# zouyilin2000/pockit

Measured on AMD Instinct MI355X. Metric: NLP-callback cycles/sec (f + grad f + g + J + H), higher is better.
Workload: dtype f64; 1 GPU; planar_quadrotor LGR 2000 intervals x 6 points (12000 nodes; n=96008, m=96000, nnz_J=755925, nnz_H=359972); inputs=guess*(1+1e-3 U) seed 0; lambda N(0,1) seed 1; sigma 1

## Files before the change

__graft_entry__.py:

```python
import os
import sys

ROOT = os.path.dirname(os.path.abspath(__file__))
if ROOT not in sys.path:
    sys.path.insert(0, ROOT)


def _bench_models():
    from pockit_amd import benchmarks as models
    import pockit_amd.radau as radau

    yield models.brachistochrone(radau, 3, 4)
    yield models.brachistochrone(radau, 200, 8)
    yield models.planar_quadrotor(radau, 2000, 6)
    yield models.two_stage_rocket(radau, 1000, 4)
    yield models.humanoid_wbc(radau, 50, 8)
    import pockit_amd.lobatto as lobatto

    yield models.planar_quadrotor(lobatto, 20, 6)
    yield models.three_stage_rocket(radau, 1000, 4)
    yield models.humanoid_team(radau, 5000, 8)


def _batch_models():
    from pockit_amd import benchmarks as models
    import pockit_amd.lobatto as lobatto
    import pockit_amd.radau as radau

    yield models.brachistochrone(radau, 3, 4)
    yield models.brachistochrone(radau, 60, 5)
    yield models.two_stage_rocket(radau, 6, 4)
    yield models.planar_quadrotor(lobatto, 20, 6)


def build() -> None:
    from pockit_amd import hipbuild, runtime
    from pockit_amd.codegen import ModelSource

    hipbuild.build_runtime(force=True)
    lib = runtime.load_library()
    for name in runtime.EXPORTS:
        getattr(lib, name)
    from pockit_amd.evaluator import compile_batched, compile_plan

    for system, _, _ in _batch_models():
        src, _ = compile_plan(system.plan)
        compile_batched(system.plan, src)
    for k, (system, _, _) in enumerate(_bench_models()):
        compile_plan(system.plan)
        if k in (2, 3, 4):
            hipbuild.compile_model(ModelSource(system.plan, sharded=True).source, fastmath=system._fastmath)
    import oracle.radau
    import subprocess

    subprocess.run([sys.executable, os.path.join(ROOT, "tools", "prune_cache.py")], check=False)


def smoke() -> None:
    import numpy as np

    from pockit_amd import benchmarks as models
    import oracle.radau
    import pockit_amd.radau as radau

    system, _, guess = models.brachistochrone(radau, 6, 5)
    ref, _, ref_guess = models.brachistochrone(oracle.radau, 6, 5)
    x, lam, sigma = models.bench_inputs(system, guess)

    def close(a, b):
        a, b = np.asarray(a), np.asarray(b)
        assert a.shape == b.shape
        assert np.max(np.abs(a - b)) <= 1e-11 * max(1.0, np.max(np.abs(b))), np.max(np.abs(a - b))

    close(system.objective(x), ref.objective(x))
    close(system.gradient(x), ref.gradient(x))
    close(system.constraints(x), ref.constraints(x))
    close(system.jacobian(x), ref.jacobian(x))
    close(system.hessian(x, lam, sigma), ref.hessian(x, lam, sigma))
    jr, jc = system.jacobianstructure()
    rr, rc = ref.jacobianstructure()
    assert np.array_equal(jr, rr) and np.array_equal(jc, rc)
    print("smoke OK: f, grad f, g, J, H of brachistochrone LGR 6x5 match the oracle on", "cuda:0")


if __name__ == "__main__":
    build()
    if len(sys.argv) > 1 and sys.argv[1] == "smoke":
        smoke()
```

pockit_amd/csrc/pk_kernels.hip.h:

```cpp
#pragma once
#include <hip/hip_runtime.h>
#include "pk_abi.h"

struct PkSys {
  const double* s;
  const double* I;
  double sigma;
  const double* lams;
};

namespace pk {

template <int G>
struct Grp {};

#define PK_CONST_AS __attribute__((address_space(4)))
typedef const int64_t PK_CONST_AS* pk_cbase_t;
__device__ __forceinline__ pk_cbase_t const_bases(const int64_t* p) { return (pk_cbase_t)(uintptr_t)p; }
__device__ __forceinline__ PkTile load_tile(const PkTile* p) {
  const int32_t PK_CONST_AS* src = (const int32_t PK_CONST_AS*)(uintptr_t)p;
  PkTile t;
  int32_t* dst = reinterpret_cast<int32_t*>(&t);
#pragma unroll
  for (int k = 0; k < (int)(sizeof(PkTile) / sizeof(int32_t)); ++k) dst[k] = src[k];
  return t;
}

template <int N>
struct SegBases {
  int lo, hi;
  pk_cbase_t mem;
  __device__ __forceinline__ void load(const int64_t* __restrict__ lb, int off, int lane) {
    mem = const_bases(lb + off);
    if (N <= PK_WAVE) {
      const long long v = lane < N ? (long long)lb[off + lane] : 0ll;
      lo = (int)v;
      hi = (int)(v >> 32);
    }
  }
  __device__ __forceinline__ void settle() {
    if (N <= PK_WAVE) asm volatile("" : "+v"(lo), "+v"(hi));
  }
  __device__ __forceinline__ int64_t operator[](int e) const {
    if (N > PK_WAVE) return mem[e];
    const unsigned l = (unsigned)__builtin_amdgcn_readlane(lo, e), h = (unsigned)__builtin_amdgcn_readlane(hi, e);
    return (int64_t)(((unsigned long long)h << 32) | l);
  }
};

template <int N>
__device__ __forceinline__ void settle(double (&v)[N]) {
#pragma unroll
  for (int i = 0; i < N; ++i) asm volatile("" : "+v"(v[i]));
}

template <int N>
__device__ __forceinline__ void fresh_args(double (&a)[N], double& tau, double& dt, double& w) {
  settle(a);
  asm volatile("" : "+v"(tau), "+v"(w));
  (void)dt;
}

__device__ __forceinline__ void loads_done() { __builtin_amdgcn_s_waitcnt(0x0F70); }

__device__ __forceinline__ void wave_lds_sync() {
  __builtin_amdgcn_fence(__ATOMIC_RELEASE, "wavefront");
  __builtin_amdgcn_wave_barrier();
  __builtin_amdgcn_fence(__ATOMIC_ACQUIRE, "wavefront");
}

#define PK_NPHASE_DIM (PK_NPHASE > 0 ? PK_NPHASE : 1)
#define PK_XCDS 8
__device__ __forceinline__ int xcd_ids_below(int n, int y) { return (n + PK_XCDS - 1 - y) / PK_XCDS; }
__device__ __forceinline__ int xcd_tile_block(int wg, int first, int total) {
  const int x = wg % PK_XCDS;
  int start = 0;
#pragma unroll
  for (int y = 0; y < PK_XCDS; ++y)
    if (y < x) start += xcd_ids_below(total, y) - xcd_ids_below(first, y);
  return start + xcd_ids_below(wg, x) - xcd_ids_below(first, x);
}

#ifdef PK_TRACE
#define PK_DIAG(bits) ((A.flags & (bits)) != 0)
#else
#define PK_DIAG(bits) false
#endif
#ifdef PK_TRACE
#define PK_TRACE_REC(role) const int pk_trec = tl.pad >= 0 ? tl.pad * 3 + (role) : -1
#define PK_MARK_AT(rec, k)                                                                                   \
  do {                                                                                                      \
    if (A.trace != nullptr && (threadIdx.x & 63) == 0 && (rec) >= 0)                                        \
      A.trace[(size_t)(rec) * 16 + (k)] = __builtin_amdgcn_s_memrealtime();                                 \
  } while (0)
#define PK_MARK(k) PK_MARK_AT(pk_trec, k)
#define PK_TRACE_PARAM , int pk_trec
#define PK_TRACE_ARG , pk_trec
#else
#define PK_TRACE_PARAM
#define PK_TRACE_ARG
#define PK_TRACE_REC(role) do { } while (0)
#define PK_MARK_AT(rec, k) do { } while (0)
#define PK_MARK(k) do { } while (0)
#endif

#ifndef PK_STREAM_FLAGS
#define PK_STREAM_FLAGS "sc1"
#endif

__device__ __forceinline__ void put(double* __restrict__ p, double v) {
  __hip_atomic_store(p, v, __ATOMIC_RELAXED, __HIP_MEMORY_SCOPE_AGENT);
}

template <int CTRL, int ROW_MASK>
__device__ __forceinline__ double dpp_take(double v) {
  const int lo = __builtin_amdgcn_update_dpp(0, __double2loint(v), CTRL, ROW_MASK, 0xf, false);
  const int hi = __builtin_amdgcn_update_dpp(0, __double2hiint(v), CTRL, ROW_MASK, 0xf, false);
  return __hiloint2double(hi, lo);
}

__device__ __forceinline__ double wave_sum(double v) {
  v += dpp_take<0xb1, 0xf>(v);
  v += dpp_take<0x4e, 0xf>(v);
  v += dpp_take<0x114, 0xf>(v);
  v += dpp_take<0x118, 0xf>(v);
  v += dpp_take<0x142, 0xa>(v);
  v += dpp_take<0x143, 0xc>(v);
  const int lo = __builtin_amdgcn_readlane(__double2loint(v), 63);
  const int hi = __builtin_amdgcn_readlane(__double2hiint(v), 63);
  return __hiloint2double(hi, lo);
}

template <int N>
__device__ __forceinline__ void wave_sums_to(double* v, double* __restrict__ dst, int lane) {
  if constexpr (N > 0) {
#pragma unroll
    for (int r = 0; r < N; ++r) v[r] = wave_sum(v[r]);
    if (lane == 0) {
#pragma unroll
      for (int r = 0; r < N; ++r) dst[r] = v[r];
    }
  }
}

#ifndef PK_BIG_MFMA
#define PK_BIG_MFMA 0
#endif
typedef double pk_d4 __attribute__((ext_vector_type(4)));
template <class Store>
__device__ __forceinline__ void mfma_rows(const double* __restrict__ Amat, int lda, int nrows, int kdim, double scale,
                                          const double* __restrict__ Bcol, int ldb, int ncols, int rb, int cb, int lane,
                                          Store&& store) {
  pk_d4 acc = {0.0, 0.0, 0.0, 0.0};
  const int arow = rb * 16 + (lane & 15), bcol = cb * 16 + (lane & 15), kq = lane >> 4;
  const bool a_ok = arow < nrows, b_ok = bcol < ncols;
  const double* __restrict__ ap = Amat + (size_t)(a_ok ? arow : 0) * lda;
  const double* __restrict__ bp = Bcol + (size_t)(b_ok ? bcol : 0) * ldb;
  for (int k0 = 0; k0 < kdim; k0 += 64) {
    double a4[4][4];
#pragma unroll
    for (int g = 0; g < 4; ++g)
#pragma unroll
      for (int u = 0; u < 4; ++u) {
        const int k = k0 + 16 * g + 4 * kq + u;
        a4[g][u] = (a_ok && k < kdim) ? ap[k] : 0.0;
      }
#pragma unroll
    for (int g = 0; g < 4; ++g) {
      if (k0 + 16 * g >= kdim) break;
      double b4[4];
#pragma unroll
      for (int u = 0; u < 4; ++u) {
        const int k = k0 + 16 * g + 4 * kq + u;
        b4[u] = (b_ok && k < kdim) ? bp[k] : 0.0;
      }
#pragma unroll
      for (int u = 0; u < 4; ++u) acc = __builtin_amdgcn_mfma_f64_16x16x4f64(a4[g][u] * scale, b4[u], acc, 0, 0, 0);
    }
  }
  if (b_ok) {
#pragma unroll
    for (int reg = 0; reg < 4; ++reg) {
      const int r = rb * 16 + kq + 4 * reg;
      if (r < nrows) store(r, bcol, acc[reg]);
    }
  }
}

#define PK_POLL_SLEEP 4
#define PK_POLL_LIMIT (1 << 24)
__device__ __forceinline__ void handoff_put(unsigned long long* slot, double v) {
  unsigned long long b = (unsigned long long)__double_as_longlong(v);
  if (b == PK_EMPTY) b = 0x7FF8000000000000ull;
  __hip_atomic_store(slot, b, __ATOMIC_RELAXED, __HIP_MEMORY_SCOPE_AGENT);
}
// ... 161 lines not shown
                                           double* acc) {
  double a[K];
#pragma unroll
  for (int c = 0; c < K; ++c) a[c] = full[c] * width * 0.5;
#pragma unroll
  for (int c = 0; c < K; ++c) {
#pragma unroll
    for (int i = 0; i < P::NX; ++i) acc[i] += a[c] * f[i * PK_WAVE + c];
  }
}

template <class P>
__device__ __forceinline__ void defect_loop(const double* __restrict__ full, const double* __restrict__ f, double width,
                                            double* acc, int K) {
#pragma unroll 4
  for (int c = 0; c < K; ++c) {
    const double a = full[c] * width * 0.5;
#pragma unroll
    for (int i = 0; i < P::NX; ++i) acc[i] += a * f[i * PK_WAVE + c];
  }
}
template <class P, int K>
__device__ __forceinline__ void defect_dot_k(const double* __restrict__ full, const double* __restrict__ f, double width,
                                             double* acc) {
  if constexpr (K * P::NX <= PK_DOT_UNROLL_MAX) defect_dot<P, K>(full, f, width, acc);
  else defect_loop<P>(full, f, width, acc, K);
}

template <class P, bool STAGED>
__device__ __forceinline__ void write_defects(const PkArgs& A, const PkPhase& ph, const PkTile& tl,
                                              const TileGeom& g, const TileTabs& T, const double* s, double dt,
                                              const double* __restrict__ fsv, const double* xr, double* xe,
                                              int lane) {
  const int nrows = tl.nj * g.R;
  if (lane >= nrows) return;
  const int jj = magic_div((uint32_t)lane, tl.magicR), r = lane - jj * g.R;
  const int endslot = tl.q0 + (jj + 1) * g.stride;
  const int back_slot = P::SCHEME ? ph.L_m - 1 : ph.L_m;
  const double* __restrict__ f = fsv + jj * g.stride;
  double acc[P::NX];
#pragma unroll
  for (int i = 0; i < P::NX; ++i) acc[i] = 0.0;
  if (STAGED) {
    const double width = T.wd[jj];
    const double* __restrict__ full = T.full + r * g.K;
    switch (g.K) {
      case 1: defect_dot_k<P, 1>(full, f, width, acc); break;
      case 2: defect_dot_k<P, 2>(full, f, width, acc); break;
      case 3: defect_dot_k<P, 3>(full, f, width, acc); break;
      case 4: defect_dot_k<P, 4>(full, f, width, acc); break;
      case 5: defect_dot_k<P, 5>(full, f, width, acc); break;
      case 6: defect_dot_k<P, 6>(full, f, width, acc); break;
      case 7: defect_dot_k<P, 7>(full, f, width, acc); break;
      case 8: defect_dot_k<P, 8>(full, f, width, acc); break;
      default:
        defect_loop<P>(full, f, width, acc, g.K);
        break;
    }
  } else {
    const double* __restrict__ full = A.db + tl.full_off + r * g.K;
    const double width = A.db[ph.width_off + tl.j0 + jj];
#pragma unroll 4
    for (int c = 0; c < g.K; ++c) {
      const double a = full[c] * width * 0.5;
#pragma unroll
      for (int i = 0; i < P::NX; ++i) acc[i] += a * f[i * PK_WAVE + c];
    }
  }
#pragma unroll
  for (int i = 0; i < P::NX; ++i) {
    if (endslot == back_slot) xe[i] = P::back_value(i, xe[i], s);
    put(&A.o_g[ph.g_off + i * ph.L_d + tl.r0 + lane], (xr[i] - xe[i]) - acc[i] * dt);
  }
}

#define PK_WIDE_NX 16
template <class P, bool STAGED, int I0, int CN, int ROW0 = I0>
__device__ __forceinline__ void defect_chunk(const PkArgs& A, const PkPhase& ph, const PkTile& tl, const TileGeom& g,
                                             const TileTabs& T, const double* s, double dt, const double* __restrict__ fsv,
                                             const double* a, int lane) {
  const int nrows = tl.nj * g.R;
  const int jj = min(magic_div((uint32_t)lane, tl.magicR), max(tl.nj - 1, 0)), r = lane - jj * g.R;
  const int src = (jj + 1) * g.stride;
  double xe[CN];
#pragma unroll
  for (int e = 0; e < CN; ++e) xe[e] = __shfl(a[I0 + e], src & (PK_WAVE - 1), PK_WAVE);
  if (lane >= nrows) return;
  if (src >= PK_WAVE) {
    const double* __restrict__ xp = A.x + ph.x_off;
#pragma unroll
    for (int e = 0; e < CN; ++e) xe[e] = xp[(I0 + e) * ph.state_len + tl.q0 + src];
  }
  const int endslot = tl.q0 + src;
  const int back_slot = P::SCHEME ? ph.L_m - 1 : ph.L_m;
  const double* __restrict__ f = fsv + jj * g.stride;
  const double* __restrict__ full = STAGED ? T.full + r * g.K : A.db + tl.full_off + r * g.K;
  const double width = STAGED ? T.wd[jj] : A.db[ph.width_off + tl.j0 + jj];
  double acc[CN];
#pragma unroll
  for (int e = 0; e < CN; ++e) acc[e] = 0.0;
#pragma unroll 4
  for (int c = 0; c < g.K; ++c) {
    const double wc = full[c] * width * 0.5;
#pragma unroll
    for (int e = 0; e < CN; ++e) acc[e] += wc * f[(ROW0 + e) * PK_WAVE + c];
  }
#pragma unroll
  for (int e = 0; e < CN; ++e) {
    if (endslot == back_slot) xe[e] = P::back_value(I0 + e, xe[e], s);
    put(&A.o_g[ph.g_off + (I0 + e) * ph.L_d + tl.r0 + lane], (a[I0 + e] - xe[e]) - acc[e] * dt);
  }
}
#define PK_TRANS_CHUNK 16
template <class P, bool STAGED, int I0>
__device__ __forceinline__ void write_translation_wide(const PkArgs& A, const PkTile& tl, const TileTabs& T,
                                                       const SegBases<P::NX>& tbase, int lane) {
  if constexpr (I0 < P::NX) {
    constexpr int CN = P::NX - I0 < PK_TRANS_CHUNK ? P::NX - I0 : PK_TRANS_CHUNK;
    const int tot = tl.nj * tl.nnzT;
    const double* __restrict__ tvg = A.db + tl.tv_off;
    double* __restrict__ run[CN];
    if constexpr (P::NX > PK_WAVE) {
      pk_cbase_t tb = tbase.mem + I0;
      asm volatile("" : "+s"(tb));
#pragma unroll
      for (int i = 0; i < CN; ++i) run[i] = A.o_jac + (tb[i] + tl.offT);
    } else {
#pragma unroll
      for (int i = 0; i < CN; ++i) run[i] = A.o_jac + (tbase[I0 + i] + tl.offT);
    }
    for (uint32_t p = lane; p < (uint32_t)tot; p += PK_WAVE) {
      const int t = (int)p - magic_div(p, tl.magicT) * tl.nnzT;
      const double v = STAGED ? T.tv[t] : tvg[t];
#pragma unroll
      for (int i = 0; i < CN; ++i) put(&run[i][p], v);
    }
    write_translation_wide<P, STAGED, I0 + PK_TRANS_CHUNK>(A, tl, T, tbase, lane);
  }
}
template <class P, bool STAGED>
__device__ __forceinline__ void write_translation(const PkArgs& A, const PkPhase& ph, const PkTile& tl,
                                                  const TileTabs& T, const SegBases<P::NX>& tbase, int lane) {
  if constexpr (P::NX > PK_WIDE_NX) return write_translation_wide<P, STAGED, 0>(A, tl, T, tbase, lane);
  const int tot = tl.nj * tl.nnzT;
  const double* __restrict__ tvg = A.db + tl.tv_off;
  double* __restrict__ run[P::NX];
#pragma unroll
  for (int i = 0; i < P::NX; ++i) run[i] = A.o_jac + (tbase[i] + tl.offT);
  for (uint32_t p = lane; p < (uint32_t)tot; p += PK_WAVE) {
    const int t = (int)p - magic_div(p, tl.magicT) * tl.nnzT;
    const double v = STAGED ? T.tv[t] : tvg[t];
#pragma unroll
    for (int i = 0; i < P::NX; ++i) put(&run[i][p], v);
  }
}

template <class P, int NI, bool HESS, bool STAGED, int E0, int S0, class Bases>
__device__ __forceinline__ void stream_loop(const PkArgs& A, const PkPhase& ph, const PkTile& tl, const TileGeom& g,
                                            const TileTabs& T, const double* __restrict__ sv,
                                            const double* __restrict__ lam_s, const Bases& bases,
                                            double* __restrict__ out, int lane) {
  double* __restrict__ run[NI > 0 ? NI : 1];
#pragma unroll
  for (int e = 0; e < NI; ++e) run[e] = out + (bases[E0 + e] + tl.offI);
  const int nnz = tl.nnzI;
  const int tot = tl.nj * nnz;
  if (STAGED) {
    typedef double pk_d2 __attribute__((ext_vector_type(2)));
    for (uint32_t p0 = 2 * lane; p0 < (uint32_t)tot; p0 += 2 * PK_WAVE) {
      double v[2][NI > 0 ? NI : 1];
      const bool pair = p0 + 1 < (uint32_t)tot;
#pragma unroll
      for (int u = 0; u < 2; ++u) {
        const uint32_t pc = (u == 0 || pair) ? p0 + u : p0;
        const int jj = magic_div(pc, tl.magicI);
        const int t = (int)pc - jj * nnz;
        const int rc = T.rc[t];
        const double val = -(T.iv[t] * T.wd[jj] * 0.5);
        const double* __restrict__ col = sv + jj * g.stride + (rc >> 16);
        const double* __restrict__ lam = lam_s + jj * g.R + (rc & 0xFFFF);
#pragma unroll
        for (int e = 0; e < NI; ++e)
          v[u][e] = HESS ? val * lam[(P::H_state(E0 + e) - S0) * PK_WAVE] * col[e * PK_WAVE] : val * col[e * PK_WAVE];
      }
#pragma unroll
      for (int e = 0; e < NI; ++e) {
        if (pair) {
          const pk_d2 w = {v[0][e], v[1][e]};
          asm volatile("global_store_dwordx4 %0, %1, off " PK_STREAM_FLAGS "\n\ts_nop 1" : : "v"(&run[e][p0]), "v"(w));
        } else {
          put(&run[e][p0], v[0][e]);
        }
      }
    }
    return;
  }
  const int32_t* __restrict__ rcg = A.ib + tl.irc_off;
  const double* __restrict__ ivg = A.db + tl.iv_off;
  const double* __restrict__ wdg = A.db + ph.width_off + tl.j0;
  for (uint32_t p = lane; p < (uint32_t)tot; p += PK_WAVE) {
    const int jj = magic_div(p, tl.magicI);
    const int t = (int)p - jj * nnz;
    const int r = rcg[2 * t], c = rcg[2 * t + 1];
    const double val = -(ivg[t] * wdg[jj] * 0.5);
    const double* __restrict__ col = sv + jj * g.stride + c;
    if (HESS) {
      const double* __restrict__ lam = lam_s + jj * g.R + r;
#pragma unroll
      for (int e = 0; e < NI; ++e) put(&run[e][p], val * lam[(P::H_state(E0 + e) - S0) * PK_WAVE] * col[e * PK_WAVE]);
    } else {
#pragma unroll
      for (int e = 0; e < NI; ++e) put(&run[e][p], val * col[e * PK_WAVE]);
    }
  }
}

template <class P, int NI, bool HESS, bool STAGED, int E0 = 0, int S0 = 0, class Bases>
__device__ __forceinline__ void stream_expanded(const PkArgs& A, const PkPhase& ph, const PkTile& tl,
                                                const TileGeom& g, const TileTabs& T, const double* __restrict__ sv,
                                                const double* __restrict__ lam_s, const Bases& segb,
                                                double* __restrict__ out, int lane) {
  if (NI == 0 || tl.nj * tl.nnzI == 0) return;
  stream_loop<P, NI, HESS, STAGED, E0, S0>(A, ph, tl, g, T, sv, lam_s, segb, out, lane);
}

#define PK_PHASE_B(T, CALL)       \
  do {                            \
    if ((T).staged) {             \
      constexpr bool STAGED = true;  \
      CALL;                       \
    } else {                      \
      constexpr bool STAGED = false; \
      CALL;                       \
    }                             \
  } while (0)

template <class P>
__device__ __forceinline__ void node_gradient_eval(const PkPhase& ph, int q, const double* a, double tau, double dt,
                                                   double w, const PkSys& sy, double* ov, double* orr, bool have_mid) {
  if (q == 0)
    P::front_grad(a, tau, dt, w, sy, nullptr, ov, orr);
  else if (P::SCHEME == 1 && q == ph.L_m - 1)
    P::back_grad(a, tau, dt, w, sy, nullptr, ov, orr);
  else if (!have_mid)
    P::mid_grad(a, tau, dt, w, sy, nullptr, ov, orr);
}

template <class P>
__device__ __forceinline__ void node_gradient_store(const PkArgs& A, const PkPhase& ph, int q, const double* ov) {
  double* __restrict__ gp = A.o_grad + ph.x_off;
#pragma unroll
  for (int i = 0; i < P::NX; ++i) put(&gp[i * ph.state_len + q], ov[i]);
#pragma unroll
  for (int i = 0; i < P::NU; ++i) put(&gp[P::NX * ph.state_len + i * ph.L_m + q], ov[P::NX + i]);
}

template <class P>
__device__ __forceinline__ void node_gradient(const PkArgs& A, const PkPhase& ph, int q, const double* a,
                                              double tau, double dt, double w, const PkSys& sy, double* ov,
                                              double* orr, bool have_mid) {
  node_gradient_eval<P>(ph, q, a, tau, dt, w, sy, ov, orr, have_mid);
  node_gradient_store<P>(A, ph, q, ov);
}

template <class P>
__device__ __forceinline__ void tile_int(const PkArgs& A, const PkTile& tl, double* __restrict__,
                                         double* __restrict__ wint, double* __restrict__, int lane) {
  if (P::INT_N == 0) return;
  const PkPhase& ph = A.ph[P::INDEX];
  const TileGeom g = tile_geom<P>(tl);
  double s[PK_NS], dt, mt;
  phase_scalars<P>(A, ph, s, dt, mt);
  double o[P::INT_N > 0 ? P::INT_N : 1];
#pragma unroll
  for (int r = 0; r < P::INT_N; ++r) o[r] = 0.0;
  if (lane < g.nown) {
    double a[P::NARG], tau, w;
    load_node<P>(A, ph, s, dt, mt, tl.q0 + lane, a, tau, w);
    P::mid_int(a, o);
#pragma unroll
    for (int r = 0; r < P::INT_N; ++r) o[r] *= w;
  }
  wave_sums_to<P::INT_N>(o, wint, lane);
}

template <class P, int C>
__device__ __forceinline__ void dyn_pass(const PkArgs& A, const PkPhase& ph, const PkTile& tl, const TileGeom& g,
                                         const TileTabs& T, const double* s, double dt, double mt,
                                         double* __restrict__ sv, int lane) {
  constexpr int I0 = P::D_c0(C), CN = P::D_cn(C);
  double a[P::NARG], tau, w;
  load_node<P>(A, ph, s, dt, mt, tl.q0 + lane, a, tau, w);
  if (lane < g.nq) {
    double o[CN];
    P::mid_dyn_g(Grp<C>{}, a, o);
#pragma unroll
    for (int e = 0; e < CN; ++e) sv[e * PK_WAVE + lane] = o[e];
  }
  wave_lds_sync();
  PK_PHASE_B(T, (defect_chunk<P, STAGED, I0, CN, 0>(A, ph, tl, g, T, s, dt, sv, a, lane)));
}
template <class P, int C = 0>
__device__ __forceinline__ void dyn_passes(const PkArgs& A, const PkPhase& ph, const PkTile& tl, const TileGeom& g,
                                           const TileTabs& T, const double* s, double dt, double mt,
                                           double* __restrict__ sv, int lane) {
  if constexpr (C < P::D_NG) {
// ... 475 lines not shown
  PK_MARK(4);
  wave_lds_sync();
  PK_MARK(5);
  if (tl.nj == 0) return;
  PK_PHASE_B(T, (stream_expanded<P, P::H_NI, true, STAGED, 0, S0>(A, ph, tl, g, T, sv, lam_s, segb, A.o_hess, lane)));
  PK_MARK(8);
#ifdef PK_TRACE
  __builtin_amdgcn_s_waitcnt(0);
  PK_MARK(9);
#endif
}

template <class P, int G>
__device__ __forceinline__ void hess_rows(const PkArgs& A, const PkPhase& ph, const PkTile& tl, double* __restrict__ lam_s,
                                          int lane) {
  constexpr int S0 = P::H_gs0(G), SN = P::H_gsn(G);
  if constexpr (P::H_gni(G) > 0 && SN > 0) {
    const int row = min(tl.r0 + lane, ph.L_d - 1);
    double lrow[SN];
#pragma unroll
    for (int i = 0; i < SN; ++i) lrow[i] = A.lam[ph.g_off + (S0 + i) * ph.L_d + row];
#pragma unroll
    for (int i = 0; i < SN; ++i) lam_s[i * PK_WAVE + lane] = lrow[i];
  }
}
template <class P, int G, bool STAGED>
__device__ __forceinline__ void hess_group_b(const PkArgs& A, const PkPhase& ph, const PkTile& tl, const TileGeom& g,
                                             const TileTabs& T, const double* __restrict__ sv,
                                             const double* __restrict__ lam_s, const SegBases<P::H_NI + P::H_NN>& segb,
                                             int lane) {
  stream_expanded<P, P::H_gni(G), true, STAGED, P::H_gi0(G), P::H_gs0(G)>(A, ph, tl, g, T, sv, lam_s, segb, A.o_hess, lane);
}
template <class P, int G, bool ONE = false>
__device__ __forceinline__ void hess_groups(const PkArgs& A, const PkPhase& ph, const PkTile& tl, const TileGeom& g,
                                            const TileTabs& T, double (&a)[P::NARG], double& tau, double& dt, double& w,
                                            const PkSys& sy, double (&lp)[P::NC > 0 ? P::NC : 1], double* __restrict__ sv,
                                            double* __restrict__ lam_s, const SegBases<P::H_NI + P::H_NN>& segb,
                                            int lane, int q, bool live, const double* s = nullptr, double mt = 0.0) {
  if constexpr (G < P::H_NG) {
    constexpr int NI = P::H_gni(G), N0 = P::H_gn0(G), NN = P::H_gnn(G);
    if constexpr (P::WIDE && !ONE) {
      hess_rows<P, G>(A, ph, tl, lam_s, lane);
      load_node<P>(A, ph, s, dt, mt, q, a, tau, w);
#pragma unroll
      for (int j = 0; j < P::NC; ++j) lp[j] = A.lam[ph.path_off + j * ph.L_m + min(q, ph.L_m - 1)];
    } else if constexpr (G > 0 && !ONE) {
      fresh_args(a, tau, dt, w);
      settle(lp);
    }
    if (live) {
      double o[NI + NN + 1];
      P::mid_hess_g(Grp<G>{}, a, tau, dt, w, sy, lp, o);
#pragma unroll
      for (int e = 0; e < NI; ++e) sv[e * PK_WAVE + lane] = o[e];
      if (NN > 0 && lane < g.nown && q >= ph.mid_lo && q < ph.mid_hi) {
#pragma unroll
        for (int e = 0; e < NN; ++e) put(&A.o_hess[segb[P::H_NI + N0 + e] + (q - ph.mid_lo)], o[NI + e]);
      }
    }
    if constexpr (NI > 0) {
      wave_lds_sync();
      if (tl.nj != 0) PK_PHASE_B(T, (hess_group_b<P, G, STAGED>(A, ph, tl, g, T, sv, lam_s, segb, lane)));
      if constexpr (!ONE) wave_lds_sync();
    }
    if constexpr (!ONE) hess_groups<P, G + 1>(A, ph, tl, g, T, a, tau, dt, w, sy, lp, sv, lam_s, segb, lane, q, live, s, mt);
  }
}

template <class P>
__device__ __forceinline__ void tile_hess_grouped(const PkArgs& A, const PkTile& tl, double* __restrict__ sv, int lane) {
  const PkPhase& ph = A.ph[P::INDEX];
  const TileGeom g = tile_geom<P>(tl);
  double s[PK_NS], dt, mt;
  phase_scalars<P>(A, ph, s, dt, mt);
  const PkSys sy{s, A.Ibuf, A.sigma, A.lam};
  SegBases<P::H_NI + P::H_NN> segb;
  segb.load(A.lb, ph.hseg_off, lane);
  double* __restrict__ lam_s = sv + P::H_GMAX * PK_WAVE;
  const bool fit = tabs_fit(A, tl, g);
  const TabRegs tr = tabs_issue(A, ph, tl, g, fit, lane);
  const int q = tl.q0 + lane;
  double a[P::NARG], tau, w, lp[P::NC > 0 ? P::NC : 1];
  if constexpr (P::WIDE) {
    const TileTabs T = tabs_commit(A, tl, g, tr, fit, lane);
    segb.settle();
    loads_done();
    wave_lds_sync();
    hess_groups<P, 0>(A, ph, tl, g, T, a, tau, dt, w, sy, lp, sv, lam_s, segb, lane, q, lane < g.nq, s, mt);
  } else {
    double lrow[P::NX];
    const int row = min(tl.r0 + lane, ph.L_d - 1);
#pragma unroll
    for (int i = 0; i < P::NX; ++i) lrow[i] = A.lam[ph.g_off + i * ph.L_d + row];
    load_node<P>(A, ph, s, dt, mt, q, a, tau, w);
#pragma unroll
    for (int j = 0; j < P::NC; ++j) lp[j] = A.lam[ph.path_off + j * ph.L_m + min(q, ph.L_m - 1)];
    const TileTabs T = tabs_commit(A, tl, g, tr, fit, lane);
#pragma unroll
    for (int i = 0; i < P::NX; ++i) lam_s[i * PK_WAVE + lane] = lrow[i];
    segb.settle();
    loads_done();
    hess_groups<P, 0>(A, ph, tl, g, T, a, tau, dt, w, sy, lp, sv, lam_s, segb, lane, q, lane < g.nq);
  }
}

template <class P>
__device__ __forceinline__ void tile_hess(const PkArgs& A, const PkTile& tl, double* __restrict__ sv,
                                          double* __restrict__, double* __restrict__, int lane) {
  if constexpr (P::H_NG == 1) tile_hess_single<P>(A, tl, sv, lane);
  else tile_hess_grouped<P>(A, tl, sv, lane);
}

template <class P, int G>
__device__ __forceinline__ void tile_hess_one(const PkArgs& A, const PkTile& tl, double* __restrict__ sv, int lane) {
  const PkPhase& ph = A.ph[P::INDEX];
  const TileGeom g = tile_geom<P>(tl);
  double s[PK_NS], dt, mt;
  phase_scalars<P>(A, ph, s, dt, mt);
  const PkSys sy{s, A.Ibuf, A.sigma, A.lam};
  SegBases<P::H_NI + P::H_NN> segb;
  segb.load(A.lb, ph.hseg_off, lane);
  double* __restrict__ lam_s = sv + P::H_GMAX * PK_WAVE;
  const bool fit = tabs_fit(A, tl, g);
  const TabRegs tr = tabs_issue(A, ph, tl, g, fit, lane);
  const int q = tl.q0 + lane;
  constexpr int S0 = P::H_gs0(G), SN = P::H_gsn(G);
  double a[P::NARG], tau, w, lp[P::NC > 0 ? P::NC : 1], lrow[SN > 0 ? SN : 1];
  const int row = min(tl.r0 + lane, ph.L_d - 1);
  constexpr bool needs_rows = P::H_gni(G) > 0;
  if (needs_rows) {
#pragma unroll
    for (int i = 0; i < SN; ++i) lrow[i] = A.lam[ph.g_off + (S0 + i) * ph.L_d + row];
  }
  load_node<P>(A, ph, s, dt, mt, q, a, tau, w);
#pragma unroll
  for (int j = 0; j < P::NC; ++j) lp[j] = A.lam[ph.path_off + j * ph.L_m + min(q, ph.L_m - 1)];
  const TileTabs T = tabs_commit(A, tl, g, tr, fit, lane);
  if (needs_rows) {
#pragma unroll
    for (int i = 0; i < SN; ++i) lam_s[i * PK_WAVE + lane] = lrow[i];
  }
  segb.settle();
  loads_done();
  hess_groups<P, G, true>(A, ph, tl, g, T, a, tau, dt, w, sy, lp, sv, lam_s, segb, lane, q, lane < g.nq);
}
template <class P, int G = 0>
__device__ __forceinline__ void tile_hess_pick(int grp, const PkArgs& A, const PkTile& tl, double* __restrict__ sv, int lane) {
  if constexpr (G < P::H_NG) {
    if (grp == G) tile_hess_one<P, G>(A, tl, sv, lane);
    else tile_hess_pick<P, G + 1>(grp, A, tl, sv, lane);
  }
}

template <class P, int ROLE, bool STAGED, bool CJ>
__device__ __forceinline__ void xall_phase_b(const PkArgs& A, const PkPhase& ph, const PkTile& tl, const TileGeom& g,
                                             const TileTabs& T, const double* s, double dt,
                                             const double* __restrict__ sv, const double* __restrict__ jsv,
                                             const double* xr, double* xe,
                                             const SegBases<P::J_NI + P::J_NN>& segb, const SegBases<P::NX>& tbase,
                                             int lane PK_TRACE_PARAM) {
  if (ROLE != 2 && !PK_DIAG(8192)) write_defects<P, STAGED>(A, ph, tl, g, T, s, dt, sv, xr, xe, lane);
  PK_MARK(6);
  if (tl.nj == 0) return;
  if (ROLE != 2 && !CJ && !PK_DIAG(16384)) write_translation<P, STAGED>(A, ph, tl, T, tbase, lane);
  PK_MARK(7);
  if (ROLE == 1) return;
  if (!PK_DIAG(32768))
    stream_expanded<P, P::J_NI, false, STAGED>(A, ph, tl, g, T, jsv, nullptr, segb, A.o_jac, lane);
}

template <class P, int ROLE, bool CJ>
__device__ __forceinline__ void tile_xall_single(const PkArgs& A, const PkTile& tl, double* __restrict__ sv,
                                                 double* __restrict__ wint, double* __restrict__ wgrad, int lane,
                                                 int pub_blk) {
  const PkPhase& ph = A.ph[P::INDEX];
  const TileGeom g = tile_geom<P>(tl);
  PK_TRACE_REC(ROLE == 2 ? 1 : 0);
  PK_MARK(0);
  double s[PK_NS], dt, mt;
  phase_scalars<P>(A, ph, s, dt, mt);
  const PkSys sy{s, A.Ibuf, A.sigma, A.lam};
  SegBases<P::J_NI + P::J_NN> segb;
  SegBases<P::NX> tbase;
  if (ROLE != 1) segb.load(A.lb, ph.jseg_off, lane);
  if (ROLE != 2) tbase.load(A.lb, ph.jt_off, lane);
  double* __restrict__ jsv = sv + P::NX * PK_WAVE;
  const bool fit = tabs_fit(A, tl, g);
  const TabRegs tr = tabs_issue(A, ph, tl, g, fit, lane);
  const int q = tl.q0 + lane;
  double a[P::NARG], tau, w, xr[P::NX], xe[P::NX];
  load_node<P>(A, ph, s, dt, mt, q, a, tau, w);
  const TileTabs T = tabs_commit(A, tl, g, tr, fit, lane);
  if (ROLE != 1) segb.settle();
  if (ROLE != 2) tbase.settle();
  PK_MARK(1);
  if (ROLE != 2) {
    defect_ends<P>(A, ph, tl, g, a, xe, lane);
    settle(xe);
  }
  loads_done();
#pragma unroll
  for (int i = 0; i < P::NX; ++i) xr[i] = a[i];
  double oi[P::INT_N > 0 ? P::INT_N : 1], orr[P::GR_NR > 0 ? P::GR_NR : 1];
#pragma unroll
  for (int r = 0; r < P::INT_N; ++r) oi[r] = 0.0;
#pragma unroll
  for (int r = 0; r < P::GR_NR; ++r) orr[r] = 0.0;
  double og[P::G_NOUT], oj[P::J_NI + P::J_NN + 1], ov[P::NX + P::NU];
  const bool live = lane < g.nq && !PK_DIAG(512);
  if (live) {
    double ot[P::GR_NR > 0 ? P::GR_NR : 1], op[P::INT_N > 0 ? P::INT_N : 1];
    PK_MARK(2);
    P::mid_xall(a, tau, dt, w, sy, og, oj, ov, ot, op);
    PK_MARK(3);
    if (ROLE != 2 && lane < g.nown) {
#pragma unroll
      for (int r = 0; r < P::INT_N; ++r) oi[r] = op[r] * w;
#pragma unroll
      for (int r = 0; r < P::GR_NR; ++r) orr[r] = ot[r];
      node_gradient_eval<P>(ph, q, a, tau, dt, w, sy, ov, orr, true);
    }
  }
  if (ROLE != 2) {
    wave_sums_to<P::INT_N>(oi, wint, lane);
    wave_sums_to<P::GR_NR>(orr, wgrad, lane);
    PK_MARK(10);
    if (pub_blk >= 0) {
      __syncthreads();
      if ((int)threadIdx.x < PK_NRED) {
        double vi = 0.0, vg = 0.0;
#pragma unroll
        for (int wv = 0; wv < PK_WAVES_PER_BLOCK; ++wv) {
          vi += wint[wv * PK_NRED + threadIdx.x];
          vg += wgrad[wv * PK_NRED + threadIdx.x];
        }
        handoff_put(A.cpart + (size_t)pub_blk * PK_NRED + threadIdx.x, vi);
        handoff_put(A.cpart2 + (size_t)pub_blk * PK_NRED + threadIdx.x, vg);
      }
      PK_MARK(11);
    }
  }
  if (live) {
    if (ROLE != 2) {
      if (lane < g.nown) node_gradient_store<P>(A, ph, q, ov);
      PK_MARK(12);
#pragma unroll
      for (int i = 0; i < P::NX; ++i) sv[i * PK_WAVE + lane] = og[i];
    }
    if (ROLE != 1) {
#pragma unroll
      for (int e = 0; e < P::J_NI; ++e) jsv[e * PK_WAVE + lane] = oj[e];
    }
    PK_MARK(13);
    if (lane < g.nown) {
      if (ROLE != 2) {
#pragma unroll
        for (int j = 0; j < P::NC; ++j) put(&A.o_g[ph.path_off + j * ph.L_m + q], og[P::NX + j]);
      }
      if (ROLE != 1 && q >= ph.mid_lo && q < ph.mid_hi) {
#pragma unroll
        for (int e = 0; e < P::J_NN; ++e) put(&A.o_jac[segb[P::J_NI + e] + (q - ph.mid_lo)], oj[P::J_NI + e]);
      }
    }
  }
  PK_MARK(4);
  wave_lds_sync();
  PK_MARK(5);
  if (PK_DIAG(256)) return;
  PK_PHASE_B(T, (xall_phase_b<P, ROLE, STAGED, CJ>(A, ph, tl, g, T, s, dt, sv, jsv, xr, xe, segb, tbase, lane PK_TRACE_ARG)));
  PK_MARK(8);
#ifdef PK_TRACE
  __builtin_amdgcn_s_waitcnt(0);
  PK_MARK(9);
#endif
}

template <class P, int ROLE, bool STAGED, bool CJ>
__device__ __forceinline__ void xval_phase_b(const PkArgs& A, const PkPhase& ph, const PkTile& tl, const TileGeom& g,
                                             const TileTabs& T, const double* s, double dt, const double* __restrict__ sv,
                                             const double* xr, double* xe, const SegBases<P::NX>& tbase, int lane) {
  if constexpr (!P::WIDE) write_defects<P, STAGED>(A, ph, tl, g, T, s, dt, sv, xr, xe, lane);
  if (!CJ && tl.nj != 0) write_translation<P, STAGED>(A, ph, tl, T, tbase, lane);
}
template <class P, int ROLE, bool CJ, bool PP = false>
__device__ __forceinline__ void tile_xall_grouped(const PkArgs& A, const PkTile& tl, double* __restrict__ sv,
                                                  double* __restrict__ wint, double* __restrict__ wgrad, int lane,
                                                  int pub_blk) {
  const PkPhase& ph = A.ph[P::INDEX];
  const TileGeom g = tile_geom<P>(tl);
  PK_TRACE_REC(ROLE == 2 ? 1 : 0);
  PK_MARK(0);
  double s[PK_NS], dt, mt;
  phase_scalars<P>(A, ph, s, dt, mt);
  const PkSys sy{s, A.Ibuf, A.sigma, A.lam};
  SegBases<P::J_NI + P::J_NN> segb;
  SegBases<P::NX> tbase;
  if (ROLE != 1) segb.load(A.lb, ph.jseg_off, lane);
  if (ROLE != 2) tbase.load(A.lb, ph.jt_off, lane);
  double* __restrict__ jsv = sv + P::XROWS * PK_WAVE;
  const bool fit = tabs_fit(A, tl, g);
  const TabRegs tr = tabs_issue(A, ph, tl, g, fit, lane);
  const int q = tl.q0 + lane;
  double a[P::NARG], tau, w;
  load_node<P>(A, ph, s, dt, mt, q, a, tau, w);
  const TileTabs T = tabs_commit(A, tl, g, tr, fit, lane);
  if (ROLE != 1) segb.settle();
  if (ROLE != 2) tbase.settle();
  loads_done();
  PK_MARK(1);
  const bool live = lane < g.nq;
  if (ROLE != 2) {
    double oi[P::INT_N > 0 ? P::INT_N : 1], orr[P::GR_NR > 0 ? P::GR_NR : 1];
#pragma unroll
    for (int r = 0; r < P::INT_N; ++r) oi[r] = 0.0;
#pragma unroll
    for (int r = 0; r < P::GR_NR; ++r) orr[r] = 0.0;
    double og[P::G_NOUT], ov[P::NX + P::NU];
    constexpr bool SUMS_FIRST = P::NX + P::NU + P::NC <= 48;
    if (live) {
      double ot[P::GR_NR > 0 ? P::GR_NR : 1], op[P::INT_N > 0 ? P::INT_N : 1];
      PK_MARK(2);
      P::mid_xval(a, tau, dt, w, sy, sv + lane, PK_WAVE, og, ov, ot, op);
      PK_MARK(3);
      if (lane < g.nown) {
#pragma unroll
        for (int r = 0; r < P::INT_N; ++r) oi[r] = op[r] * w;
#pragma unroll
        for (int r = 0; r < P::GR_NR; ++r) orr[r] = ot[r];
        node_gradient_eval<P>(ph, q, a, tau, dt, w, sy, ov, orr, true);
        if constexpr (!SUMS_FIRST) {
          node_gradient_store<P>(A, ph, q, ov);
#pragma unroll
          for (int j = 0; j < P::NC; ++j) put(&A.o_g[ph.path_off + j * ph.L_m + q], og[P::NX + j]);
        }
      }
    }
    PK_MARK(12);
    wave_sums_to<P::INT_N>(oi, wint, lane);
    wave_sums_to<P::GR_NR>(orr, wgrad, lane);
    PK_MARK(10);
    if (pub_blk >= 0) {
      __syncthreads();
      if ((int)threadIdx.x < PK_NRED) {
        double vi = 0.0, vg = 0.0;
#pragma unroll
        for (int wv = 0; wv < PK_WAVES_PER_BLOCK; ++wv) {
          vi += wint[wv * PK_NRED + threadIdx.x];
// ... 1946 lines not shown
```

pockit_amd/hipbuild.py:

```python
from __future__ import annotations

import hashlib
import os
import shutil
import subprocess
import tempfile

HERE = os.path.dirname(os.path.abspath(__file__))
CSRC = os.path.join(HERE, "csrc")
LIB_PATH = os.path.join(HERE, "libpockit_hip.so")
CACHE_DIR = os.environ.get("POCKIT_AMD_CACHE", os.path.join(HERE, "_cache"))
ARCH = "gfx950"


def _hipcc():
    exe = shutil.which("hipcc") or "/opt/rocm/bin/hipcc"
    if not os.path.exists(exe):
        raise RuntimeError("hipcc not found: the MI355X evaluator needs the ROCm toolchain to build its kernels")
    return exe


def _run(cmd):
    res = subprocess.run(cmd, capture_output=True, text=True)
    if res.returncode != 0:
        errs = [ln for ln in res.stderr.splitlines() if "error" in ln.lower() and "remark:" not in ln]
        raise RuntimeError("command failed: " + " ".join(cmd) + "\n" + "\n".join(errs[:20]) + "\n...\n" + res.stderr[-3000:])
    return res


def _stale(target, sources):
    if not os.path.exists(target):
        return True
    t = os.path.getmtime(target)
    return any(os.path.getmtime(s) > t for s in sources)


RUNTIME_SOURCES = [os.path.join(CSRC, name) for name in
                   ("pk_runtime.cpp", "pk_shim.cpp", "pk_pool.cpp", "pk_shard.cpp", "pk_batch.cpp", "pk_extras.cpp", "pk_ops.cpp", "pk_merit.cpp", "pk_error.cpp")]
POOL_SOURCES = [os.path.join(CSRC, name) for name in ("pk_pool.cpp", "pk_error.cpp")]
RUNTIME_HEADERS = [os.path.join(CSRC, name) for name in
                   ("pk_runtime.h", "pk_error.h", "pockit_hip_internal.h", "pk_abi.h", "pk_launch.h")] + [
                       os.path.join(os.path.dirname(HERE), "include", "pockit_hip.h")]


def build_runtime(force=False):
    if force or _stale(LIB_PATH, RUNTIME_SOURCES + RUNTIME_HEADERS):
        _run([_hipcc(), f"--offload-arch={ARCH}", "-O2", "-fPIC", "-shared", "-std=c++17"] + RUNTIME_SOURCES + ["-o", LIB_PATH])
    return LIB_PATH


EXTRA_FLAGS = os.environ.get("POCKIT_AMD_HIPCC_FLAGS", "").split()


PRELOAD_FLAGS = ["-mllvm", "-amdgpu-kernarg-preload-count=4"]


def _kernel_header_hash():
    h = hashlib.sha256()
    for name in ("pk_kernels.hip.h", "pk_abi.h"):
        with open(os.path.join(CSRC, name), "rb") as fh:
            h.update(fh.read())
    return h.hexdigest()[:12]


def live_keys():
    cur, keep = _kernel_header_hash(), set()
    if os.path.isdir(CACHE_DIR):
        for name in os.listdir(CACHE_DIR):
            if name.endswith(".gen"):
                try:
                    with open(os.path.join(CACHE_DIR, name)) as fh:
                        if fh.read().strip() == cur:
                            keep.add(name[:-4])
                except OSError:
                    pass
    return keep


def write_index(keep):
    if os.path.isdir(CACHE_DIR):
        for name in os.listdir(CACHE_DIR):
            if name.endswith(".gen") and name[:-4] not in keep:
                os.remove(os.path.join(CACHE_DIR, name))


def _parse_resource_usage(stderr: str) -> dict:
    keys = {"TotalSGPRs": "sgpr", "SGPRs": "sgpr", "VGPRs": "vgpr", "AGPRs": "agpr", "ScratchSize [bytes/lane]": "scratch",
            "Occupancy [waves/SIMD]": "occupancy", "SGPRs Spill": "sgpr_spill", "VGPRs Spill": "vgpr_spill",
            "LDS Size [bytes/block]": "lds"}
    out, cur = {}, None
    for line in stderr.splitlines():
        if "remark:" not in line:
            continue
        body = line.split("remark:", 1)[1].split("[-Rpass-analysis")[0].strip()
        if body.startswith("Function Name:"):
            cur = out.setdefault(body.split(":", 1)[1].strip(), {})
            continue
        if cur is None or ":" not in body:
            continue
        name, val = body.rsplit(":", 1)
        if name.strip() in keys:
            try:
                cur[keys[name.strip()]] = int(val.strip())
            except ValueError:
                pass
    return out


def resource_usage(source: str, fastmath: bool = False, extra_flags=()):
    import json

    path = os.path.join(CACHE_DIR, _key(source, fastmath, extra_flags) + ".res.json")
    if not os.path.exists(path):
        return None
    with open(path) as fh:
        return json.load(fh)


def spills(usage) -> dict:
    return {k: (v.get("vgpr_spill", 0), v.get("scratch", 0)) for k, v in (usage or {}).items() if v.get("vgpr_spill", 0) > 0}


def _key(source: str, fastmath: bool, extra_flags=()) -> str:
    return hashlib.sha256((source + _kernel_header_hash() + str(bool(fastmath)) + " ".join(PRELOAD_FLAGS + EXTRA_FLAGS + list(extra_flags))
                           ).encode()).hexdigest()[:32]


COMPILE_SECONDS = {"total": 0.0, "count": 0, "last": 0.0}


def compile_model(source: str, fastmath: bool = False, keep_source: bool = None, extra_flags=()) -> bytes:
    if keep_source is None:
        keep_source = os.environ.get("POCKIT_AMD_KEEP_SOURCE", "0") == "1"
    import zlib

    key = _key(source, fastmath, extra_flags)
    os.makedirs(CACHE_DIR, exist_ok=True)
    path = os.path.join(CACHE_DIR, key + ".hsacoz")
    gen = os.path.join(CACHE_DIR, key + ".gen")
    if os.path.exists(path) and not os.path.exists(gen):
        try:
            with open(gen, "w") as fh:
                fh.write(_kernel_header_hash())
        except OSError:
            pass
    if not os.path.exists(path):
        import time

        t_start = time.perf_counter()
        with tempfile.TemporaryDirectory() as tmp:
            src = os.path.join(tmp, "model.hip")
            with open(src, "w") as fh:
                fh.write(source)
            cmd = [_hipcc(), f"--offload-arch={ARCH}", "-O3", "-std=c++17", "--genco", f"-I{CSRC}", src, "-o",
                   os.path.join(tmp, "model.hsaco"), "-Rpass-analysis=kernel-resource-usage"] + PRELOAD_FLAGS + EXTRA_FLAGS + list(extra_flags)
            if fastmath:
                cmd += ["-fassociative-math", "-freciprocal-math", "-fno-signed-zeros", "-fno-trapping-math"]
            res = _run(cmd)
            try:
                import json

                fd, staged = tempfile.mkstemp(dir=CACHE_DIR, prefix=key + ".", suffix=".part")
                with os.fdopen(fd, "w") as fh:
                    json.dump(_parse_resource_usage(res.stderr), fh)
                os.replace(staged, os.path.join(CACHE_DIR, key + ".res.json"))
            except OSError:
                pass
            fd, staged = tempfile.mkstemp(dir=CACHE_DIR, prefix=key + ".", suffix=".part")
            with open(os.path.join(tmp, "model.hsaco"), "rb") as fin, os.fdopen(fd, "wb") as fout:
                fout.write(zlib.compress(fin.read(), 6))
            os.replace(staged, path)
            if keep_source:
                fd, staged = tempfile.mkstemp(dir=CACHE_DIR, prefix=key + ".", suffix=".part")
                os.close(fd)
                shutil.copyfile(src, staged)
                os.replace(staged, os.path.join(CACHE_DIR, key + ".hip"))
            with open(gen, "w") as fh:
                fh.write(_kernel_header_hash())
        COMPILE_SECONDS["last"] = time.perf_counter() - t_start
        COMPILE_SECONDS["total"] += COMPILE_SECONDS["last"]
        COMPILE_SECONDS["count"] += 1
        log = os.environ.get("POCKIT_AMD_COMPILE_LOG")
        if log:
            try:
                with open(log, "a") as fh:
                    fh.write(f"{key} {COMPILE_SECONDS['last']:.1f}\n")
            except OSError:
                pass
    used = os.environ.get("POCKIT_AMD_USED_LOG")
    if used:
        try:
            with open(used, "a") as fh:
                fh.write(key + "\n")
        except OSError:
            pass
    with open(path, "rb") as fh:
        return zlib.decompress(fh.read())
```

Baseline: 221,100 cycles/s.

## Distribute translation-block Jacobian writes across a block's waves as one run

Adds a values-run descriptor that detects when the four tiles of a block form a contiguous run with identical structure. When they do, the translation-value writes are redistributed: each wave handles 128-position chunks across all states of the combined run and uses paired dwordx4 stores instead of per-tile strided loops. The run metadata is parked in spare lanes of the SegBases register so it survives to phase B. This costs extra tile-metadata loads and validation per block, and it depends on the pub_blk and scheme conditions holding.

```diff
diff --git a/__graft_entry__.py b/__graft_entry__.py
--- a/__graft_entry__.py
+++ b/__graft_entry__.py
@@ -31,6 +31,7 @@
     yield models.brachistochrone(radau, 60, 5)
     yield models.two_stage_rocket(radau, 6, 4)
     yield models.planar_quadrotor(lobatto, 20, 6)
+    yield models.planar_quadrotor(radau, 44, 6)
 
 
 def build() -> None:
diff --git a/pockit_amd/csrc/pk_kernels.hip.h b/pockit_amd/csrc/pk_kernels.hip.h
--- a/pockit_amd/csrc/pk_kernels.hip.h
+++ b/pockit_amd/csrc/pk_kernels.hip.h
@@ -1,6 +1,7 @@
 #pragma once
 #include <hip/hip_runtime.h>
 #include "pk_abi.h"
+#include "pk_values_run.h"
 
 struct PkSys {
   const double* s;
@@ -41,6 +42,11 @@
   __device__ __forceinline__ void settle() {
     if (N <= PK_WAVE) asm volatile("" : "+v"(lo), "+v"(hi));
   }
+  __device__ __forceinline__ void park(int lane, int v0, int v1) {
+    static_assert(N <= PK_WAVE - 2, "no free lanes");
+    lo = lane == PK_WAVE - 1 ? v0 : (lane == PK_WAVE - 2 ? v1 : lo);
+  }
+  __device__ __forceinline__ int parked(int slot) const { return __builtin_amdgcn_readlane(lo, PK_WAVE - 1 - slot); }
   __device__ __forceinline__ int64_t operator[](int e) const {
     if (N > PK_WAVE) return mem[e];
     const unsigned l = (unsigned)__builtin_amdgcn_readlane(lo, e), h = (unsigned)__builtin_amdgcn_readlane(hi, e);
@@ -508,6 +514,30 @@
     const double v = STAGED ? T.tv[t] : tvg[t];
 #pragma unroll
     for (int i = 0; i < P::NX; ++i) put(&run[i][p], v);
+  }
+}
+
+template <class P, bool STAGED>
+__device__ __forceinline__ void translation_by_run(const PkArgs& A, const PkTile& tl, const TileTabs& T,
+                                                   const SegBases<P::NX>& tbase, const PkValuesRun& vr, int lane) {
+  typedef double pk_d2 __attribute__((ext_vector_type(2)));
+  const double* __restrict__ tvg = A.db + tl.tv_off;
+  const int wave = __builtin_amdgcn_readfirstlane(threadIdx.x >> 6);
+  const int npos = pk_run_npos(vr), nw = pk_run_nw(vr), chunks = pk_run_chunks(npos);
+  for (PkRunUnit u = pk_run_first(wave, chunks); u.state < P::NX; pk_run_next(u, nw, chunks)) {
+    double* __restrict__ run = A.o_jac + (tbase[u.state] + vr.offT);
+    const uint32_t p0 = (uint32_t)pk_run_pos(u.chunk, lane);
+    const int cnt = pk_run_count((int)p0, npos);
+    if (cnt == 0) continue;
+    const int t0 = (int)p0 - magic_div(p0, tl.magicT) * tl.nnzT;
+    const int t1 = t0 + 1 == tl.nnzT ? 0 : t0 + 1;
+    const double v0 = STAGED ? T.tv[t0] : tvg[t0];
+    if (cnt == 2) {
+      const pk_d2 w = {v0, STAGED ? T.tv[t1] : tvg[t1]};
+      asm volatile("global_store_dwordx4 %0, %1, off " PK_STREAM_FLAGS "\n\ts_nop 1" : : "v"(&run[p0]), "v"(w));
+    } else {
+      put(&run[p0], v0);
+    }
   }
 }
 
@@ -1289,6 +1319,21 @@
   }
 }
 
+__device__ __forceinline__ PkValuesRun block_values_run(const PkTile* tiles, int n_tiles, int blk, const PkTile& own) {
+  static_assert(PK_RUN_TILES == PK_WAVES_PER_BLOCK && PK_RUN_LANES == PK_WAVE, "pk_values_run.h restates pk_abi.h");
+  const int t0 = blk * PK_WAVES_PER_BLOCK;
+  if (t0 + PK_WAVES_PER_BLOCK > n_tiles) return pk_run_none();
+  const PkTile PK_CONST_AS* src = (const PkTile PK_CONST_AS*)(uintptr_t)(tiles + t0);
+  PkRunTile t[PK_RUN_TILES];
+#pragma unroll
+  for (int w = 0; w < PK_RUN_TILES; ++w)
+    t[w] = PkRunTile{own.phase, src[w].kid, src[w].kidf, own.K, src[w].nj, src[w].q0, src[w].r0, src[w].offT, own.nnzT};
+  return pk_values_run(t);
+}
+
+template <class P, int ROLE, bool CJ>
+__device__ constexpr bool values_by_run() { return ROLE == 1 && !CJ && P::NX <= PK_WIDE_NX; }
+
 template <class P, int ROLE, bool STAGED, bool CJ>
 __device__ __forceinline__ void xall_phase_b(const PkArgs& A, const PkPhase& ph, const PkTile& tl, const TileGeom& g,
                                              const TileTabs& T, const double* s, double dt,
@@ -1299,7 +1344,12 @@
   if (ROLE != 2 && !PK_DIAG(8192)) write_defects<P, STAGED>(A, ph, tl, g, T, s, dt, sv, xr, xe, lane);
   PK_MARK(6);
   if (tl.nj == 0) return;
-  if (ROLE != 2 && !CJ && !PK_DIAG(16384)) write_translation<P, STAGED>(A, ph, tl, T, tbase, lane);
+  if (ROLE != 2 && !CJ && !PK_DIAG(16384)) {
+    PkValuesRun vrun = pk_run_none();
+    if constexpr (values_by_run<P, ROLE, CJ>()) vrun = PkValuesRun{tbase.parked(0), (uint32_t)tbase.parked(1)};
+    if (pk_run_nw(vrun) > 0 && pk_run_scheme(vrun) == P::SCHEME) translation_by_run<P, STAGED>(A, tl, T, tbase, vrun, lane);
+    else write_translation<P, STAGED>(A, ph, tl, T, tbase, lane);
+  }
   PK_MARK(7);
   if (ROLE == 1) return;
   if (!PK_DIAG(32768))
@@ -1327,9 +1377,16 @@
   const int q = tl.q0 + lane;
   double a[P::NARG], tau, w, xr[P::NX], xe[P::NX];
   load_node<P>(A, ph, s, dt, mt, q, a, tau, w);
+  PkValuesRun vrun = pk_run_none();
+  if constexpr (values_by_run<P, ROLE, CJ>()) {
+    const PkTile* tiles = A.tile;
+    const int n_tiles = A.n_tiles;
+    if (pub_blk >= 0) vrun = block_values_run(tiles, n_tiles, pub_blk, tl);
+  }
   const TileTabs T = tabs_commit(A, tl, g, tr, fit, lane);
   if (ROLE != 1) segb.settle();
   if (ROLE != 2) tbase.settle();
+  if constexpr (values_by_run<P, ROLE, CJ>()) tbase.park(lane, vrun.offT, (int)vrun.bits);
   PK_MARK(1);
   if (ROLE != 2) {
     defect_ends<P>(A, ph, tl, g, a, xe, lane);
diff --git a/pockit_amd/csrc/pk_values_run.h b/pockit_amd/csrc/pk_values_run.h
--- /dev/null
+++ b/pockit_amd/csrc/pk_values_run.h
@@ -0,0 +1,82 @@
+#pragma once
+#include <stdint.h>
+
+#if defined(__HIPCC__)
+#define PK_RUN_FN __host__ __device__ inline
+#else
+#define PK_RUN_FN inline
+#endif
+
+#define PK_RUN_TILES 4
+#define PK_RUN_LANES 64
+#define PK_RUN_CHUNK 128
+#define PK_RUN_MAX_POS 65536
+
+struct PkRunTile {
+  int32_t phase, kid, kidf, K, nj, q0, r0, offT, nnzT;
+};
+
+struct PkValuesRun {
+  int32_t offT;
+  uint32_t bits;
+};
+PK_RUN_FN PkValuesRun pk_run_make(int nw, int offT, int npos, int scheme) {
+  const PkValuesRun r = {offT, (uint32_t)npos | (uint32_t)nw << 16 | (uint32_t)scheme << 20};
+  return r;
+}
+PK_RUN_FN PkValuesRun pk_run_none() { return pk_run_make(0, 0, 0, 0); }
+PK_RUN_FN int pk_run_npos(const PkValuesRun& r) { return (int)(r.bits & 0xFFFFu); }
+PK_RUN_FN int pk_run_nw(const PkValuesRun& r) { return (int)(r.bits >> 16 & 0xFu); }
+PK_RUN_FN int pk_run_scheme(const PkValuesRun& r) { return (int)(r.bits >> 20 & 1u); }
+
+PK_RUN_FN PkValuesRun pk_values_run(const PkRunTile (&t)[PK_RUN_TILES]) {
+  int nw = 0;
+  bool ok = true;
+#pragma unroll
+  for (int w = 0; w < PK_RUN_TILES; ++w) {
+    const bool has = t[w].nj > 0;
+    ok = ok && !(has && nw != w);
+    nw += has ? 1 : 0;
+  }
+  ok = ok && nw == PK_RUN_TILES && t[0].K <= PK_RUN_LANES && t[0].nnzT > 0;
+  const int scheme = t[1].q0 - t[0].q0 == t[0].nj * t[0].K ? 0 : 1;
+  int npos = t[0].nj * t[0].nnzT;
+#pragma unroll
+  for (int w = 0; w < PK_RUN_TILES; ++w)
+    if (w < nw) ok = ok && t[w].nj * (t[w].K - scheme) + scheme < PK_RUN_LANES;
+#pragma unroll
+  for (int w = 1; w < PK_RUN_TILES; ++w) {
+    if (w < nw) {
+      const PkRunTile &a = t[w - 1], &b = t[w];
+      const int step = a.nj * (a.K - scheme);
+      ok = ok && b.phase == a.phase && b.kid == a.kid && b.kidf == a.kidf && b.K == a.K && b.nnzT == a.nnzT &&
+           b.q0 == a.q0 + step && b.r0 == a.r0 + step && b.offT == a.offT + a.nj * a.nnzT;
+      npos += b.nj * b.nnzT;
+    }
+  }
+  ok = ok && npos < PK_RUN_MAX_POS;
+  return ok ? pk_run_make(nw, t[0].offT, npos, scheme) : pk_run_none();
+}
+
+PK_RUN_FN int pk_run_chunks(int npos) { return (npos + PK_RUN_CHUNK - 1) / PK_RUN_CHUNK; }
+
+struct PkRunUnit {
+  int32_t state, chunk;
+};
+PK_RUN_FN PkRunUnit pk_run_first(int w, int chunks) {
+  PkRunUnit u = {0, w};
+  while (u.chunk >= chunks) {
+    u.chunk -= chunks;
+    ++u.state;
+  }
+  return u;
+}
+PK_RUN_FN void pk_run_next(PkRunUnit& u, int nw, int chunks) {
+  u.chunk += nw;
+  while (u.chunk >= chunks) {
+    u.chunk -= chunks;
+    ++u.state;
+  }
+}
+PK_RUN_FN int pk_run_pos(int chunk, int lane) { return chunk * PK_RUN_CHUNK + 2 * lane; }
+PK_RUN_FN int pk_run_count(int p0, int npos) { return p0 + 1 < npos ? 2 : (p0 < npos ? 1 : 0); }
diff --git a/pockit_amd/hipbuild.py b/pockit_amd/hipbuild.py
--- a/pockit_amd/hipbuild.py
+++ b/pockit_amd/hipbuild.py
@@ -57,7 +57,7 @@
 
 def _kernel_header_hash():
     h = hashlib.sha256()
-    for name in ("pk_kernels.hip.h", "pk_abi.h"):
+    for name in ("pk_kernels.hip.h", "pk_abi.h", "pk_values_run.h"):
         with open(os.path.join(CSRC, name), "rb") as fh:
             h.update(fh.read())
     return h.hexdigest()[:12]
```

Result: slower. 160,200 cycles/s (-27.5%).
